# facebook/facebook360_dep

Hardware: AMD Instinct MI355X
Metric: depth Mpix/s per GPU (full pyramid, 16-cam 2048^2 rig); % HBM-read roofline (higher is better)
Workload: dtype f32+f64; 1 GPU; BASELINE config 3: 16-camera 2048x2048 synthetic rig, 8-frame sequence, full 10-level pyramid per frame, per-level temporal filter (+-2 frames); the same sequence for every --gpus N (block partition, 8 frame(s) on this rank); rig=cfg2, cameras=16, frames=8, temporal_filter=True, halo_transport=local, parallelism=frames x1

## Files before the change

facebook360_dep_amd/csrc/derp_camera.h:

```cpp
#pragma once
#include <hip/hip_runtime.h>
#include <math.h>
#include <stdint.h>

#include "../../include/derp_hip.h"

#define DERP_HD __host__ __device__ __forceinline__

namespace derp {

struct Cam {
  double pos[3];
  double R[9];
  double principal[2];
  double focal[2];
  double dist[3];
  double dist_max;
  double cos_fov;
  double edge_sq;
  int32_t type;
  int32_t default_fov;
  int32_t dist_zero;
  int32_t pad;
};

struct D2 {
  double x, y;
};
struct D3 {
  double x, y, z;
};

DERP_HD double sum3(double a, double b, double c) {
  return a + (b + c);
}

DERP_HD double distort_factor(const Cam& c, double r2) {
  double result = c.dist[2];
  result = c.dist[1] + r2 * result;
  result = c.dist[0] + r2 * result;
  return 1.0 + r2 * result;
}
DERP_HD double distort(const Cam& c, double r) {
  r = (c.dist_max < r) ? c.dist_max : r;
  return distort_factor(c, r * r) * r;
}

DERP_HD double undistort(const Cam& c, const double y) {
  if (c.dist_zero) {
    return y;
  }
  if (y >= distort(c, c.dist_max)) {
    return c.dist_max;
  }
  const double smidgen = 1.0 / 1e4;
  double x0 = 0, y0 = 0, dy0 = 1;
  for (int step = 0; step < 10; ++step) {
    const double x1 = (y - y0) / dy0 + x0;
    const double y1 = distort(c, x1);
    if (fabs(y1 - y) < smidgen) {
      return x1;
    }
    const double dy1 = (distort(c, x1 + smidgen) - y1) / smidgen;
    x0 = x1;
    y0 = y1;
    dy0 = dy1;
  }
  return x0;
}

static constexpr int kAtanLutDoubles = 20;
#if defined(__HIP_DEVICE_COMPILE__)
__device__ __forceinline__ double div_plain(double n, double d) {
  double r = __builtin_amdgcn_rcp(d);
  r = __builtin_fma(__builtin_fma(-d, r, 1.0), r, r);
  r = __builtin_fma(__builtin_fma(-d, r, 1.0), r, r);
  const double q = n * r;
// ... 145 lines not shown
    if (p.z < 0) {
      const double n = DERP_SQRT(sum3(p.x * p.x, p.y * p.y, p.z * p.z));
      px = p.x / n;
      py = p.y / n;
    } else {
      const double n = DERP_SQRT(p.x * p.x + p.y * p.y);
      px = p.x / n;
      py = p.y / n;
    }
    const double f = distort_factor(c, px * px + py * py);
    return {f * px, f * py};
  }
}

#undef DERP_SQRT
DERP_HD D3 sensor_to_camera(const Cam& c, const D2& s) {
  const double sq = s.x * s.x + s.y * s.y;
  if (sq == 0) {
    return {0, 0, -1};
  }
  const double norm = sqrt(sq);
  const double r = undistort(c, norm);
  double theta;
  if (c.type == DERP_FTHETA) {
    theta = r;
  } else if (c.type == DERP_RECTILINEAR) {
    theta = atan(r);
  } else if (c.type == DERP_EQUISOLID) {
    theta = r <= 2 ? 2 * asin(r / 2) : M_PI;
  } else {
    theta = r <= 1 ? asin(r) : M_PI / 2;
  }
  const double k = sin(theta) / norm;
  return {k * s.x, k * s.y, -cos(theta)};
}

DERP_HD D3 rig_direction(const Cam& c, double px, double py, double prx, double pry, double fx, double fy) {
  const D2 sensor = {(px - prx) / fx, (py - pry) / fy};
  const D3 u = sensor_to_camera(c, sensor);
  return {
      sum3(c.R[0] * u.x, c.R[3] * u.y, c.R[6] * u.z),
      sum3(c.R[1] * u.x, c.R[4] * u.y, c.R[7] * u.z),
      sum3(c.R[2] * u.x, c.R[5] * u.y, c.R[8] * u.z)};
}

DERP_HD bool outside_image_circle(const Cam& c, double px, double py, double prx, double pry, double fx, double fy) {
  if (c.default_fov) {
    return false;
  }
  const double sx = (px - prx) / fx, sy = (py - pry) / fy;
  return sx * sx + sy * sy >= c.edge_sq;
}

template <int LEAN = 0>
DERP_HD bool sees(const Cam& c, const D3& rig, double prx, double pry, double fx, double fy,
                  double resx, double resy, D2& pix, const double* atanLut = nullptr) {
  const D3 v = {rig.x - c.pos[0], rig.y - c.pos[1], rig.z - c.pos[2]};
  const double back = sum3(c.R[6] * v.x, c.R[7] * v.y, c.R[8] * v.z);
  if (c.cos_fov != -1) {
    if (c.cos_fov == 0) {
      if (back >= 0) {
        return false;
      }
    } else {
      const double dot = -back;
      const double sq = sum3(v.x * v.x, v.y * v.y, v.z * v.z);
      if (dot * fabs(dot) <= c.cos_fov * fabs(c.cos_fov) * sq) {
        return false;
      }
    }
  }
  const D3 cam = {
      sum3(c.R[0] * v.x, c.R[1] * v.y, c.R[2] * v.z),
      sum3(c.R[3] * v.x, c.R[4] * v.y, c.R[5] * v.z),
      back};
  const D2 s = camera_to_sensor<LEAN>(c, cam, atanLut);
  pix.x = fx * s.x + prx;
  pix.y = fy * s.y + pry;
  return !(0 > pix.x || pix.x >= resx || 0 > pix.y || pix.y >= resy);
}

inline double host_poly(const double* k, int deg, double x) {
  double acc = k[deg];
  for (int i = deg; i-- > 0;) {
    acc = acc * x + k[i];
  }
  return acc;
}

inline double host_smallest_positive_root(const double* k, int deg) {
  double stops[4];
  int n_stops = 0;
  if (deg == 3) {
    const double a = 3 * k[3], b = 2 * k[2], c = k[1];
    const double disc = b * b - 4 * a * c;
    if (disc >= 0) {
      const double q = -0.5 * (b + copysign(sqrt(disc), b));
      double r0 = q / a, r1 = (q != 0) ? c / q : r0;
      if (r0 > r1) {
        const double t = r0;
        r0 = r1;
        r1 = t;
      }
      if (r0 > 0) {
        stops[n_stops++] = r0;
      }
      if (r1 > 0 && r1 != r0) {
        stops[n_stops++] = r1;
      }
    }
  } else if (deg == 2) {
    const double r = -k[1] / (2 * k[2]);
    if (r > 0) {
      stops[n_stops++] = r;
    }
  }
  double left = 0, f_left = k[0];
  for (int seg = 0; seg <= n_stops; ++seg) {
    double right;
    if (seg < n_stops) {
      right = stops[seg];
    } else {
// ... 121 lines not shown
    c.R[3] = t + sz;
    t = c1x * az;
    c.R[2] = t + sy;
    c.R[6] = t - sy;
    t = c1y * az;
    c.R[5] = t - sx;
    c.R[7] = t + sx;
    c.R[0] = c1x * ax + cs;
    c.R[4] = c1y * ay + cs;
    c.R[8] = c1z * az + cs;
  }
  double res[2] = {j.resolution[0], j.resolution[1]};
  double pr[2] = {j.has_principal ? j.principal[0] : res[0] / 2, j.has_principal ? j.principal[1] : res[1] / 2};
  c.dist[0] = c.dist[1] = c.dist[2] = 0;
  c.dist_max = INFINITY;
  if (j.has_distortion) {
    int count = 3;
    while (count > 0 && j.distortion[count - 1] == 0) {
      --count;
    }
    if (count > 0) {
      double k[4] = {1, 0, 0, 0};
      for (int i = 0; i < count; ++i) {
        k[i + 1] = j.distortion[i] * (2 * i + 3);
      }
      const double y = host_smallest_positive_root(k, count);
      for (int i = 0; i < 3; ++i) {
        c.dist[i] = j.distortion[i];
      }
      c.dist_max = sqrt(y);
    }
  }
  c.dist_zero = (c.dist[0] == 0 && c.dist[1] == 0 && c.dist[2] == 0);
  const double def_cos = (j.type == DERP_RECTILINEAR || j.type == DERP_ORTHOGRAPHIC) ? 0.0 : -1.0;
  if (j.has_fov) {
    c.cos_fov = cos(j.fov);
    if (!(c.cos_fov >= def_cos)) {
      return "fov exceeds the camera type's default";
    }
  } else {
    c.cos_fov = def_cos;
  }
  c.default_fov = (c.cos_fov == def_cos);
  c.principal[0] = pr[0] / res[0];
  c.principal[1] = pr[1] / res[1];
  c.focal[0] = j.focal[0] / res[0];
  c.focal[1] = j.focal[1] / res[1];
  c.edge_sq = 0;
  if (!c.default_fov) {
    const double sin_fov = sqrt(1 - c.cos_fov * c.cos_fov);
    const D2 e = camera_to_sensor(c, D3{0, sin_fov, -c.cos_fov});
    c.edge_sq = e.x * e.x + e.y * e.y;
  }
  c.pad = 0;
  return nullptr;
}

}
```

facebook360_dep_amd/csrc/derp_capi.hip:

```cpp
#include <hip/hip_runtime.h>

#include <algorithm>
#include <cfloat>
#include <cmath>
#include <cstdarg>
#include <cstdio>
#include <cstdlib>
#include <cstring>
#include <map>
#include <memory>
#include <string>
#include <vector>

#include <rocprim/device/device_radix_sort.hpp>

#include "../../include/derp_hip.h"
#include "derp_host.h"
#include "derp_kernels.h"
#include "derp_mesh.h"
#include "derp_points.h"
#include "derp_render.h"
#include "derp_geometric.h"
#include "derp_sweep.h"
#include "derp_align.h"
// ... 1073 lines not shown
  (void)hipMemcpy(c->camsSrc.p, c->camsSrcH.data(), sizeof(Cam) * n_src, hipMemcpyHostToDevice);
  (void)hipMemcpy(c->camsDst.p, c->camsDstH.data(), sizeof(Cam) * n_dst, hipMemcpyHostToDevice);
  (void)hipMemcpy(c->dst2src.p, c->dst2srcH.data(), sizeof(int) * n_dst, hipMemcpyHostToDevice);
  (void)hipMemset(c->counters.p, 0, c->counters.bytes);
  *out = owner.release();
  return 0;
}

void derp_destroy(derp_ctx* c) {
  if (!c) {
    return;
  }
  (void)hipSetDevice(c->device);
  (void)hipStreamSynchronize(c->stream);
  for (auto& l : c->lanes) {
    (void)hipStreamSynchronize(l->stream);
  }
  drain_spans(c);
  for (auto& l : c->lanes) {
    (void)hipStreamDestroy(l->stream);
    (void)hipEventDestroy(l->done);
  }
  if (c->laneReady) {
    (void)hipEventDestroy(c->laneReady);
  }
  (void)hipStreamDestroy(c->stream);
  (void)hipStreamDestroy(c->copyStream);
  delete c;
}

const char* derp_last_error(const derp_ctx* c) {
  return c ? c->err.c_str() : g_create_error.c_str();
}

int derp_set_options(derp_ctx* c, const derp_options* o) {
  if (!c || !o) {
    return 1;
  }
  if (o->random_proposals < 0) {
    return fail(c, "Check failed: random_proposals >= 0");
  }
  c->opt = *o;
  return 0;
}

int derp_set_pyramid(derp_ctx* c, int num_levels, const int* widths, const int* heights, int width_full,
                     int height_full) {
  if (!c) {
    return 1;
  }
  if (num_levels <= 0 || num_levels > kMaxLevels) {
    return fail(c, "num_levels %d out of range (1..%d)", num_levels, kMaxLevels);
  }
  HIPCHK(c, hipSetDevice(c->device));
  c->numLevels = num_levels;
  c->widthFull = width_full;
  c->heightFull = height_full;
  c->LW.assign(widths, widths + num_levels);
  c->LH.assign(heights, heights + num_levels);
  c->frames.clear();
  c->frames.resize(1);
  c->curSlot = 0;
  TRY(alloc_pyramid(c, c->frame()));
  size_t nmax = 0;
  for (int l = 0; l < num_levels; ++l) {
    nmax = std::max(nmax, npx(c, l));
  }
  TRY(alloc_work_set(c, c->w, nmax));
  ALLOC(c, c->fovMask, nmax * c->D);
  c->cur = -1;
  c->warpCachedLevel = -1;
  c->fovCachedLevel = -1;
  HIPCHK(c, hipStreamSynchronize(c->stream));
  return 0;
}

int derp_set_frame_slots(derp_ctx* c, int n_slots) {
  if (!c || c->numLevels == 0) {
    return fail(c, "derp_set_pyramid has not been called");
  }
  if (n_slots < 1 || n_slots > 4096) {
    return fail(c, "n_slots %d out of range (1..4096)", n_slots);
  }
  HIPCHK(c, hipSetDevice(c->device));
  TRY(select_frame(c, 0));
  const int had = (int)c->frames.size();
  c->frames.resize(n_slots);
  for (int k = had; k < n_slots; ++k) {
    TRY(alloc_pyramid(c, c->frames[k]));
  }
  HIPCHK(c, hipStreamSynchronize(c->stream));
  return 0;
}

int derp_select_frame(derp_ctx* c, int slot) {
  if (!c || c->numLevels == 0) {
    return fail(c, "derp_set_pyramid has not been called");
  }
  return select_frame(c, slot);
}

int derp_frame_slots(const derp_ctx* c, int* n_slots, int* selected) {
  if (!c) {
    return 1;
  }
  if (n_slots) {
// ... 327 lines not shown
```

facebook360_dep_amd/csrc/derp_debug_api.h:

```cpp
#pragma once

namespace {
struct HostPairs {
  SsdPair* p;
  SsdPair get(int i) const {
    return p[i];
  }
  void set(int i, const SsdPair& v) {
    p[i] = v;
  }
};
int stage_index(const char* stage) {
  for (int i = 0; i < ST_COUNT; ++i) {
    if (strcmp(stage, kStageNames[i]) == 0) {
      return i;
    }
  }
  return -1;
}
}

int derp_debug_atan2_ypos(derp_ctx* c, const double* y, const double* x, double* out, size_t n) {
  if (!c || !y || !x || !out) {
    return fail(c, "bad arguments");
  }
  ALLOC(c, c->w.staging, 3 * n * sizeof(double));
  double* d = c->w.staging.as<double>();
  HIPCHK(c, hipMemcpyAsync(d, y, n * sizeof(double), hipMemcpyHostToDevice, c->stream));
  HIPCHK(c, hipMemcpyAsync(d + n, x, n * sizeof(double), hipMemcpyHostToDevice, c->stream));
  hipLaunchKernelGGL(k_debug_atan2_ypos, dim3(flat_grid(n)), dim3(256), 0, c->stream, d, d + n, d + 2 * n, n);
  KCHECK(c);
  HIPCHK(c, hipMemcpyAsync(out, d + 2 * n, n * sizeof(double), hipMemcpyDeviceToHost, c->stream));
  HIPCHK(c, hipStreamSynchronize(c->stream));
  return 0;
}

int derp_debug_fp64(derp_ctx* c, int op, const double* a, const double* b, double* out, size_t n) {
  if (!c || !a || !out || op < 0 || op > 3 || (op >= 2 && !b)) {
    return fail(c, "bad arguments");
  }
  if (n == 0) {
    return 0;
  }
  ALLOC(c, c->w.staging, 3 * n * sizeof(double));
  double* d = c->w.staging.as<double>();
  HIPCHK(c, hipMemcpyAsync(d, a, n * sizeof(double), hipMemcpyHostToDevice, c->stream));
  HIPCHK(c, hipMemcpyAsync(d + n, op >= 2 ? b : a, n * sizeof(double), hipMemcpyHostToDevice, c->stream));
  hipLaunchKernelGGL(k_debug_fp64, dim3(flat_grid(n)), dim3(256), 0, c->stream, op, d, d + n, d + 2 * n, n);
  KCHECK(c);
  HIPCHK(c, hipMemcpyAsync(out, d + 2 * n, n * sizeof(double), hipMemcpyDeviceToHost, c->stream));
  HIPCHK(c, hipStreamSynchronize(c->stream));
  return 0;
}

int derp_debug_expf(derp_ctx* c, int mode, const float* x, float* out, size_t n) {
  if (!c || !x || !out || mode < 0 || mode > 1) {
    return fail(c, "bad arguments");
  }
  if (n == 0) {
    return 0;
  }
  ALLOC(c, c->w.staging, 2 * n * sizeof(float));
  float* d = c->w.staging.as<float>();
  HIPCHK(c, hipMemcpyAsync(d, x, n * sizeof(float), hipMemcpyHostToDevice, c->stream));
  hipLaunchKernelGGL(k_debug_expf, dim3(flat_grid(n)), dim3(256), 0, c->stream, mode, d, d + n, n);
  KCHECK(c);
  HIPCHK(c, hipMemcpyAsync(out, d + n, n * sizeof(float), hipMemcpyDeviceToHost, c->stream));
  HIPCHK(c, hipStreamSynchronize(c->stream));
  return 0;
}

int derp_debug_sees(derp_ctx* c, int src, const double* xyz, size_t n, double* out) {
  if (!c || !xyz || !out || src < 0 || src >= c->S) {
    return fail(c, "bad arguments");
  }
  if (n == 0) {
    return 0;
  }
  ALLOC(c, c->w.staging, 9 * n * sizeof(double));
  double* d = c->w.staging.as<double>();
  HIPCHK(c, hipMemcpyAsync(d, xyz, 3 * n * sizeof(double), hipMemcpyHostToDevice, c->stream));
  hipLaunchKernelGGL(k_debug_sees, dim3(flat_grid(n)), dim3(256), 0, c->stream, c->camsSrc.as<Cam>(), src, d, d + 3 * n, n);
  KCHECK(c);
  HIPCHK(c, hipMemcpyAsync(out, d + 3 * n, 6 * n * sizeof(double), hipMemcpyDeviceToHost, c->stream));
  HIPCHK(c, hipStreamSynchronize(c->stream));
  return 0;
}

int derp_debug_download(derp_ctx* c, int d, int s, int which, void* out) {
  TRY(need_current(c, false));
  const int L = c->cur;
  const int W = c->LW[L], H = c->LH[L];
  const size_t n = (size_t)W * H;
  HIPCHK(c, hipStreamSynchronize(c->stream));
  if (which == 4) {
    HIPCHK(c, hipMemcpy(out, c->w.srcVar.as<float>() + (size_t)s * n, n * sizeof(float), hipMemcpyDeviceToHost));
    return 0;
  }
  if (which == 5) {
    HIPCHK(c, hipMemcpy(out, c->fovMask.as<uint8_t>() + (size_t)d * n, n, hipMemcpyDeviceToHost));
    return 0;
  }
  if (which == 9) {
    if (s < 0 || s >= c->S) {
      return fail(c, "bad source index");
    }
    std::vector<ushort4> tmp(n);
    HIPCHK(c, hipMemcpy(tmp.data(), c->w.ownBias.as<ushort4>() + (size_t)s * n, n * sizeof(ushort4), hipMemcpyDeviceToHost));
    uint16_t* o = reinterpret_cast<uint16_t*>(out);
// ... 286 lines not shown
```

facebook360_dep_amd/csrc/derp_kernels.h:

```cpp
#pragma once
#include <hip/hip_runtime.h>
#include <math.h>
#include <stdint.h>

#include <type_traits>

#include "derp_camera.h"
#include "gcc_algos.h"

namespace derp {

#ifndef DERP_COST_MIN_WAVES
#define DERP_COST_MIN_WAVES 4
#endif
#ifndef DERP_RANDOM_MIN_WAVES
#define DERP_RANDOM_MIN_WAVES 4
#endif
#ifndef DERP_RANDOM_TILED
#define DERP_RANDOM_TILED 0
#endif
#ifndef DERP_MIX_HOT_ONLY
#define DERP_MIX_HOT_ONLY 0
#endif
#ifndef DERP_PHASE_TIMERS
// ... 159 lines not shown

struct LdsPairs {
  SsdPair* base;
  int stride;
  const double* atanLut;
  __device__ __forceinline__ SsdPair get(int i) const {
    return base[i * stride];
  }
  __device__ __forceinline__ void set(int i, const SsdPair& v) {
    base[i * stride] = v;
  }
};

__device__ __forceinline__ LdsPairs cost_wave_prologue(const LevelView& V, int d, int x0, int y0, PatchWin*& win) {
  extern __shared__ SsdPair ldsPairs[];
  __shared__ PatchWin patchWin[kCostBlock / 64];
  win = &patchWin[threadIdx.x >> 6];
  patch_window_fill(V, V.dst2src[d], x0, y0, win);
#if defined(__HIP_DEVICE_COMPILE__)
  __shared__ double atanLut[kAtanLutDoubles];
  atan_lut_fill(atanLut);
  LdsPairs pairs{ldsPairs + threadIdx.x, (int)blockDim.x, atanLut};
#else
  LdsPairs pairs{ldsPairs + threadIdx.x, (int)blockDim.x, nullptr};
#endif
  __syncthreads();
  return pairs;
}
__device__ __forceinline__ LdsPairs cost_block_prologue(PatchWin*& win) {
  static_assert(kCostBlock == 64, "a wave leaves an empty tile on its own: the block must be that one wave");
  extern __shared__ SsdPair ldsPairs[];
  __shared__ PatchWin patchWin[kCostBlock / 64];
  win = &patchWin[threadIdx.x >> 6];
#if defined(__HIP_DEVICE_COMPILE__)
  __shared__ double atanLut[kAtanLutDoubles];
  return LdsPairs{ldsPairs + threadIdx.x, (int)blockDim.x, atanLut};
#else
  return LdsPairs{ldsPairs + threadIdx.x, (int)blockDim.x, nullptr};
#endif
}
__device__ __forceinline__ void cost_tile_prologue(const LevelView& V, int d, int x0, int y0, PatchWin* win, const LdsPairs& pairs,
                                                   bool& lutReady) {
  __syncthreads();
  patch_window_fill(V, V.dst2src[d], x0, y0, win);
#if defined(__HIP_DEVICE_COMPILE__)
  if (!lutReady) {
    atan_lut_fill(const_cast<double*>(pairs.atanLut));
    lutReady = true;
  }
#endif
  __syncthreads();
}

struct SsdTexels {
  u4a8 raw[4][2];
  u4a8 ba, bb;
};
template <bool TILED>
__device__ __forceinline__ void ssd_issue_random(const LevelView& V, const ushort4* __restrict__ col, const ushort4* __restrict__ colT,
                                                 const ushort4* __restrict__ bia, float xDstSrc, float yDstSrc, SsdTexels& T,
                                                 bool& border) {
  const int pitch = V.W + 2 * kPadC;
  const int xi = (int)roundf(xDstSrc), yi = (int)roundf(yDstSrc);
  const unsigned off = ((unsigned)(yi - 2 + kPadC) * (unsigned)pitch + (unsigned)(xi - 2 + kPadC)) * 8u;
  if constexpr (TILED) {
    const unsigned xa = (unsigned)(xi - 2 + kPadC), ya = (unsigned)(yi - 2 + kPadC);
    const unsigned rowTiles = (unsigned)tiled_tiles_x(V.W) * 128u;
    const unsigned xr = xa & 3u, yr = ya & 3u;
    const unsigned base0 = (ya >> 2) * rowTiles + (xa >> 2) * 128u + yr * 32u + xr * 8u;
    const char* base = reinterpret_cast<const char*>(colT);
    typedef unsigned int u2 __attribute__((ext_vector_type(2)));
#pragma unroll
    for (int row = 0; row < 4; ++row) {
      const unsigned ro = base0 + (unsigned)row * 32u + ((yr + (unsigned)row > 3u) ? rowTiles - 128u : 0u);
#pragma unroll
      for (int k = 0; k < 4; ++k) {
        const unsigned o = ro + (unsigned)k * 8u + ((xr + (unsigned)k > 3u) ? 96u : 0u);
        const u2 t = *reinterpret_cast<const u2*>(base + o);
        if (k & 1) {
          T.raw[row][k >> 1].z = t.x;
          T.raw[row][k >> 1].w = t.y;
        } else {
          T.raw[row][k >> 1].x = t.x;
          T.raw[row][k >> 1].y = t.y;
        }
      }
    }
  } else {
    const char* base = reinterpret_cast<const char*>(col);
#pragma unroll
    for (int row = 0; row < 4; ++row) {
      T.raw[row][0] = *reinterpret_cast<const u4a8*>(base + (off + (unsigned)row * (unsigned)pitch * 8u));
      T.raw[row][1] = *reinterpret_cast<const u4a8*>(base + (off + (unsigned)row * (unsigned)pitch * 8u + 16u));
    }
  }
  border = xi < 2 || yi < 2 || xi > V.W - 2 || yi > V.H - 2;
  T.ba = T.bb = (u4a8){0u, 0u, 0u, 0u};
  if (border) {
    const unsigned boff = off + ((unsigned)pitch + 1u) * 8u;
    const char* bbase = reinterpret_cast<const char*>(bia);
    T.ba = *reinterpret_cast<const u4a8*>(bbase + boff);
    T.bb = *reinterpret_cast<const u4a8*>(bbase + (boff + (unsigned)pitch * 8u));
  }
}
__device__ __forceinline__ void ssd_issue(const LevelView& V, const ushort4* __restrict__ col,
                                          const ushort4* __restrict__ bia, float xDstSrc, float yDstSrc, SsdTexels& T) {
  const int pitch = V.W + 2 * kPadC;
  const int xi = (int)roundf(xDstSrc), yi = (int)roundf(yDstSrc);
  const unsigned off = ((unsigned)(yi - 2 + kPadC) * (unsigned)pitch + (unsigned)(xi - 2 + kPadC)) * 8u;
  const char* base = reinterpret_cast<const char*>(col);
#pragma unroll
  for (int row = 0; row < 4; ++row) {
    T.raw[row][0] = *reinterpret_cast<const u4a8*>(base + (off + (unsigned)row * (unsigned)pitch * 8u));
    T.raw[row][1] = *reinterpret_cast<const u4a8*>(base + (off + (unsigned)row * (unsigned)pitch * 8u + 16u));
  }
  const unsigned boff = off + ((unsigned)pitch + 1u) * 8u;
  const char* bbase = reinterpret_cast<const char*>(bia);
  T.ba = *reinterpret_cast<const u4a8*>(bbase + boff);
  T.bb = *reinterpret_cast<const u4a8*>(bbase + (boff + (unsigned)pitch * 8u));
}

template <bool RANDOM>
__device__ __forceinline__ SsdPair ssd_arith(const LevelView& V, const PixCtx& px, const ushort4* __restrict__ col,
                                             const SsdTexels& T, float xDstSrc, float yDstSrc, bool border = true) {
  const int pitch = V.W + 2 * kPadC;
  const u4a8 (&raw)[4][2] = T.raw;
  auto word_bg = [&](const u4a8 (&q)[4][2], int r, int k) { return (k & 1) ? q[r][k >> 1].z : q[r][k >> 1].x; };
  auto word_r = [&](const u4a8 (&q)[4][2], int r, int k) { return (k & 1) ? q[r][k >> 1].w : q[r][k >> 1].y; };
  float bias[3];
  const float bxf = roundf(xDstSrc), byf = roundf(yDstSrc);
  const float bxw = xDstSrc - bxf + 0.5f, byw = yDstSrc - byf + 0.5f;
  const float w00 = (1 - bxw) * (1 - byw), w01 = bxw * (1 - byw), w10 = (1 - bxw) * byw, w11 = bxw * byw;
  if constexpr (RANDOM) {
    float top[3][2], bot[3][2];
#pragma unroll
    for (int k = 3; k >= 0; --k) {
      float c[3][4];
#pragma unroll
      for (int r = 0; r < 4; ++r) {
        const unsigned bg = word_bg(raw, r, k), rr = word_r(raw, r, k);
        c[0][r] = (float)(bg & 0xffff);
        c[1][r] = (float)(bg >> 16);
        c[2][r] = (float)(rr & 0xffff);
      }
#pragma unroll
      for (int ch = 0; ch < 3; ++ch) {
        const float m = c[ch][1] + c[ch][2];
        const float vT = m + c[ch][0], vB = m + c[ch][3];
        if (k == 3) {
          top[ch][1] = vT + 4.0f;
          bot[ch][1] = vB + 4.0f;
        } else if (k == 2) {
          top[ch][1] += vT;
          bot[ch][1] += vB;
          top[ch][0] = vT + 4.0f;
          bot[ch][0] = vB + 4.0f;
        } else if (k == 1) {
          top[ch][1] += vT;
          bot[ch][1] += vB;
          top[ch][0] += vT;
          bot[ch][0] += vB;
        } else {
          top[ch][0] += vT;
          bot[ch][0] += vB;
        }
      }
    }
    const float ninth = 1.0f / 9.0f;
#pragma unroll
    for (int ch = 0; ch < 3; ++ch) {
      const float t00 = __builtin_truncf(top[ch][0] * ninth), t01 = __builtin_truncf(top[ch][1] * ninth);
      const float t10 = __builtin_truncf(bot[ch][0] * ninth), t11 = __builtin_truncf(bot[ch][1] * ninth);
      bias[ch] = px.dstBias(ch) - bilerp_u16(t00, t01, t10, t11, w00, w01, w10, w11);
    }
    if (__ballot(border) != 0ull) {
      if (border) {
        const u4a8 a = T.ba, b = T.bb;
        bias[0] = px.dstBias(0) - bilerp_u16((float)(a.x & 0xffff), (float)(a.z & 0xffff), (float)(b.x & 0xffff), (float)(b.z & 0xffff), w00, w01, w10, w11);
        bias[1] = px.dstBias(1) - bilerp_u16((float)(a.x >> 16), (float)(a.z >> 16), (float)(b.x >> 16), (float)(b.z >> 16), w00, w01, w10, w11);
        bias[2] = px.dstBias(2) - bilerp_u16((float)(a.y & 0xffff), (float)(a.w & 0xffff), (float)(b.y & 0xffff), (float)(b.w & 0xffff), w00, w01, w10, w11);
      }
    }
  } else {
// ... 72 lines not shown
    const v2f biasBG = (v2f){bias[0], bias[1]};
    const v2f omyp = splat2(1.0f) - ywp;
    const float omym = 1 - ywm;
    ColF lo, hi;
    unpack(0, lo);
#pragma unroll
    for (int ix = 0; ix < 3; ++ix) {
      unpack(ix + 1, hi);
      const float omx = 1 - xw[ix];
      const v2f w00p = splat2(omx) * omyp, w01p = splat2(xw[ix]) * omyp, w10p = splat2(omx) * ywp, w11p = splat2(xw[ix]) * ywp;
      const float w00m = omx * omym, w01m = xw[ix] * omym, w10m = omx * ywm, w11m = xw[ix] * ywm;
      float bgd0[3], bgd1[3];
#pragma unroll
      for (int iy = 0; iy < 3; ++iy) {
        const float w00 = iy == 1 ? w00m : iy == 0 ? w00p.x : w00p.y;
        const float w01 = iy == 1 ? w01m : iy == 0 ? w01p.x : w01p.y;
        const float w10 = iy == 1 ? w10m : iy == 0 ? w10p.x : w10p.y;
        const float w11 = iy == 1 ? w11m : iy == 0 ? w11p.x : w11p.y;
        const v2f v = splat2(w00) * lo.bg[iy] + splat2(w01) * hi.bg[iy] + splat2(w10) * lo.bg[iy + 1] +
                      splat2(w11) * hi.bg[iy + 1];
        const v2f db = px.patchBG(ix, iy) - trunc2(v);
        const v2f dn = db - biasBG;
        const v2f s0 = db * db, s1 = dn * dn;
        float t0 = s0.x + s0.y, t1 = s1.x + s1.y;
        asm("" : "+v"(t0), "+v"(t1));
        bgd0[iy] = t0;
        bgd1[iy] = t1;
      }
      v2f e0, e1;
      {
        const v2f v = w00p * lo.rE + w01p * hi.rE + w10p * lo.rO + w11p * hi.rO;
        const v2f db = (v2f){px.patchR(ix, 0), px.patchR(ix, 2)} - trunc2(v);
        const v2f dn = db - splat2(bias[2]);
        e0 = (v2f){bgd0[0], bgd0[2]} + db * db;
        e1 = (v2f){bgd1[0], bgd1[2]} + dn * dn;
      }
      float m0, m1;
      {
        const float v = w00m * lo.rO.x + w01m * hi.rO.x + w10m * lo.rE.y + w11m * hi.rE.y;
        const float db = px.patchR(ix, 1) - __builtin_truncf(v);
        const float dn = db - bias[2];
        m0 = bgd0[1] + db * db;
        m1 = bgd1[1] + dn * dn;
      }
      first += e0.x;
      first += m0;
      first += e0.y;
      second += e1.x;
      second += m1;
      second += e1.y;
      lo = hi;
    }
  };
  const float xfc = roundf(xDstSrc), yfc = roundf(yDstSrc);
  const bool exact = (xDstSrc >= 1.0f) && (yDstSrc >= 1.0f) && ((xDstSrc + 1.0f) - 1.0f == xDstSrc) &&
                     ((yDstSrc + 1.0f) - 1.0f == yDstSrc);
  int xi[3], yi[3];
  float xw[3], yw[3];
  bool regular = true;
  xi[1] = (int)xfc;
  yi[1] = (int)yfc;
  xw[0] = xw[1] = xw[2] = xDstSrc - xfc + 0.5f;
  yw[0] = yw[1] = yw[2] = yDstSrc - yfc + 0.5f;
  if (!exact) {
#pragma unroll
    for (int k = 0; k < 3; k += 2) {
      const float xs = xDstSrc + (float)(k - 1), ys = yDstSrc + (float)(k - 1);
      const float xf = roundf(xs), yf = roundf(ys);
      xi[k] = (int)xf;
      yi[k] = (int)yf;
      xw[k] = xs - xf + 0.5f;
      yw[k] = ys - yf + 0.5f;
    }
    regular = (xi[0] == xi[1] - 1) && (xi[2] == xi[1] + 1) && (yi[0] == yi[1] - 1) && (yi[2] == yi[1] + 1);
  }
  if (!RANDOM && __ballot(!exact) == 0ull) {
    const float xwu[3] = {xw[1], xw[1], xw[1]};
    block_packed(xwu, splat2(yw[1]), yw[1]);
  } else if (regular) {
    if constexpr (RANDOM) {
      block_scalar(xw, yw);
    } else {
      block_packed(xw, (v2f){yw[0], yw[2]}, yw[1]);
    }
  } else if (DERP_MIX_HOT_ONLY) {
    first = second = 0.f;
  } else {
    for (int ix = 0; ix < 3; ++ix) {
      for (int iy = 0; iy < 3; ++iy) {
        const float w00 = (1 - xw[ix]) * (1 - yw[iy]), w01 = xw[ix] * (1 - yw[iy]);
        const float w10 = (1 - xw[ix]) * yw[iy], w11 = xw[ix] * yw[iy];
        const int x0 = min(max(xi[ix] - 1, -kPadC), V.W + kPadC - 1), x1 = min(max(xi[ix], -kPadC), V.W + kPadC - 1);
        const int y0 = min(max(yi[iy] - 1, -kPadC), V.H + kPadC - 1), y1 = min(max(yi[iy], -kPadC), V.H + kPadC - 1);
        const ushort4 q00 = col[(size_t)(y0 + kPadC) * pitch + x0 + kPadC];
        const ushort4 q01 = col[(size_t)(y0 + kPadC) * pitch + x1 + kPadC];
        const ushort4 q10 = col[(size_t)(y1 + kPadC) * pitch + x0 + kPadC];
        const ushort4 q11 = col[(size_t)(y1 + kPadC) * pitch + x1 + kPadC];
        const float p00[3] = {(float)q00.x, (float)q00.y, (float)q00.z};
        const float p01[3] = {(float)q01.x, (float)q01.y, (float)q01.z};
        const float p10[3] = {(float)q10.x, (float)q10.y, (float)q10.z};
        const float p11[3] = {(float)q11.x, (float)q11.y, (float)q11.z};
        const v2f pbg = px.winBG[iy * kWinW + ix];
        const float pch[3] = {pbg.x, pbg.y, px.winR[iy * kWinW + ix]};
        float d0 = 0.f, d1 = 0.f;
        for (int c = 0; c < 3; ++c) {
          const float cs = bilerp_u16(p00[c], p01[c], p10[c], p11[c], w00, w01, w10, w11);
          const float db = pch[c] - cs;
// ... 95 lines not shown
  if constexpr (RELOAD_RAY) {
    unsigned i = pix;
    asm("" : "+v"(i) : "v"(disparity));
    const double* rd = V.rayDir + (size_t)(V.dst0 + dl) * ((size_t)V.W * V.H);
    if constexpr (RANDOM) {
      rayD = {at32(rd, i), at32(rd + V.rayStride, i), at32(rd + 2 * V.rayStride, i)};
    } else {
      rayD = {rd[i], rd[V.rayStride + i], rd[2 * V.rayStride + i]};
    }
  }
  const D3 pWorld = {px.rayO.x + rayD.x * depth, px.rayO.y + rayD.y * depth, px.rayO.z + rayD.z * depth};
  const size_t wPlane = warp_plane(V), cPlane = color_plane(V);
  const int wPitch = V.W + 2 * kPadW;
  unsigned mask = 0, waveMask = 0;
  cull = __builtin_amdgcn_readfirstlane(__ballot(!(depth >= kCullMinDepth)) != 0ull ? 0u : cull);
  const ushort4* colBase = V.projColor + (size_t)dl * (V.S - 1) * cPlane;
  const ushort4* biaBase = V.projBias + (size_t)dl * (V.S - 1) * cPlane;
  const size_t tPlane = tiled_plane(V.W, V.H);
  const ushort4* colTBase = RANDOM ? V.projColorT + (size_t)dl * (V.S - 1) * tPlane : nullptr;
  {
    bool pend = false;
    int pendSlot = 0;
    f4a8 pa = {0, 0, 0, 0}, pb = {0, 0, 0, 0};
    float pxw = 0, pyw = 0;
    auto consume = [&]() {
      const float w00 = (1 - pxw) * (1 - pyw), w01 = pxw * (1 - pyw), w10 = (1 - pxw) * pyw, w11 = pxw * pyw;
      const float wx = bilerp_f(pa.x, pa.z, pb.x, pb.z, w00, w01, w10, w11);
      const float wy = bilerp_f(pa.y, pa.w, pb.y, pb.w, w00, w01, w10, w11);
      const float xDstSrc = wx + 0.5f, yDstSrc = wy + 0.5f;
      const bool ok = pend && !(isnan(xDstSrc) || isnan(yDstSrc));
      if (ok) {
        pairs.set(pendSlot, SsdPair{xDstSrc, yDstSrc});
        mask |= 1u << pendSlot;
      }
      if (__ballot(ok) != 0ull) {
        waveMask |= 1u << pendSlot;
      }
    };
    for (int s = 0; s < V.S; ++s) {
      if (s == own || ((cull >> slot(s, own)) & 1u)) {
        continue;
      }
      const Cam& cs = V.camsSrc[s];
      D2 pn;
      const bool vis = sees<cost_sees_lean<RANDOM>()>(cs, pWorld, cs.principal[0], cs.principal[1], cs.focal[0], cs.focal[1],
                                                      1.0, 1.0, pn, pairs.atanLut);
      if (__ballot(pend) != 0ull) {
        consume();
      }
      pend = vis;
      pendSlot = slot(s, own);
      if (__ballot(vis) != 0ull) {
        const float sx = (float)(pn.x * V.Wd), sy = (float)(pn.y * V.Hd);
        const float xf = roundf(sx), yf = roundf(sy);
        const int xi = (int)xf, yi = (int)yf;
        pxw = sx - xf + 0.5f;
        pyw = sy - yf + 0.5f;
        const size_t tab = (size_t)dl * (V.S - 1) + pendSlot;
        const char* wbase = reinterpret_cast<const char*>(V.projWarp + tab * wPlane);
        const unsigned woff = vis ? ((unsigned)(yi - 1 + kPadW) * (unsigned)wPitch + (unsigned)(xi - 1 + kPadW)) * 8u : 0u;
        pa = *reinterpret_cast<const f4a8*>(wbase + woff);
        pb = *reinterpret_cast<const f4a8*>(wbase + (woff + (unsigned)wPitch * 8u));
      }
    }
    if (__ballot(pend) != 0ull) {
      consume();
    }
  }
  const unsigned tc1 = phase_clock();
  const int ssdCount = __popc(mask);
  nPair += ssdCount;
#ifdef DERP_COUNT_UNION
  if (slots) {
    *slots += __popc(__builtin_amdgcn_readfirstlane(waveMask));
  }
#endif
  int keep = 1;
  if (ssdCount < keep) {
    return make_float2(3.402823466e+38f, 0.0f);
  }
  {
    int cnt = 0;
    for (unsigned wm = __builtin_amdgcn_readfirstlane(waveMask); wm != 0; wm &= wm - 1) {
      const int t = __builtin_ctz(wm);
      if ((mask >> t) & 1) {
        const SsdPair e = pairs.get(t);
        const SsdPair ssd = compute_ssd<RANDOM>(V, px, colBase + (size_t)t * cPlane, biaBase + (size_t)t * cPlane, e.first,
                                                        e.second, RANDOM ? colTBase + (size_t)t * tPlane : nullptr);
        pairs.set(cnt, ssd);
        ++cnt;
      }
    }
  }
  const unsigned tc2 = phase_clock();
  keep = max(keep, ssdCount - 2);
  GccSelect<LdsPairs> sel(pairs);
  sel.nth_element(keep, ssdCount);
  float cost = 0;
  for (int i = 0; i < keep; ++i) {
    cost += pairs.get(i).second;
  }
  cost /= (float)keep;
  const float trustCoef = 1.0f / (float)keep;
  float confidence = px.confidence;
  if constexpr (RELOAD_RAY) {
    unsigned i = pix;
    asm("" : "+v"(i) : "v"(cost));
// ... 1365 lines not shown
__device__ __forceinline__ float expf_glibc_poly(float x, const unsigned long long* tab) {
  const double InvLn2N = 0x1.71547652b82fep+0 * 32;
  const double C0 = 0x1.c6af84b912394p-5 / 32 / 32 / 32, C1 = 0x1.ebfce50fac4f3p-3 / 32 / 32,
               C2 = 0x1.62e42ff0c52d6p-1 / 32;
  const double SHIFT = 0x1.8p+52;
  const double xd = (double)x;
  double kd = __builtin_fma(InvLn2N, xd, SHIFT);
  const unsigned long long ki = (unsigned long long)__double_as_longlong(kd);
  kd -= SHIFT;
  const double r = __builtin_fma(InvLn2N, xd, -kd);
  const unsigned long long t = tab[ki & 31] + (ki << 47);
  const double sc = __longlong_as_double((long long)t);
  const double z = __builtin_fma(C0, r, C1);
  const double r2 = r * r;
  double y = __builtin_fma(C2, r, 1.0);
  y = __builtin_fma(z, r2, y);
  y = y * sc;
  return (float)y;
}

__device__ __forceinline__ float expf_glibc(float x, const unsigned long long* tab) {
  const unsigned abstop = (__float_as_uint(x) >> 20) & 0x7ff;
  if (abstop >= (0x42b00000u >> 20)) {
    if (__float_as_uint(x) == 0xff800000u) {
      return 0.0f;
    }
    if (abstop >= (0x7f800000u >> 20)) {
      return x + x;
    }
    if (x > 0x1.62e42ep6f) {
      return __builtin_inff();
    }
    if (x < -0x1.9fe368p6f) {
      return 0.0f;
    }
  }
  return expf_glibc_poly(x, tab);
}

__device__ __forceinline__ float expf_glibc_nonpos(float x, const unsigned long long* tab) {
  if (x < -0x1.9fe368p6f) {
    return 0.0f;
  }
  return expf_glibc_poly(x, tab);
}

__global__ void __launch_bounds__(256) k_debug_expf(int mode, const float* __restrict__ x, float* __restrict__ out, size_t n) {
  __shared__ unsigned long long expTab[32];
  if (threadIdx.x < 32) {
    expTab[threadIdx.x] = kExp2fTab[threadIdx.x];
  }
  __syncthreads();
  for (size_t i = (size_t)blockIdx.x * blockDim.x + threadIdx.x; i < n; i += (size_t)gridDim.x * blockDim.x) {
    out[i] = mode == 0 ? expf_glibc(x[i], expTab) : expf_glibc_nonpos(x[i], expTab);
  }
}

template <bool GUIDE_U16>
__device__ __forceinline__ float4 bilateral_texel(const void* __restrict__ guideV, size_t j, float value) {
  if (GUIDE_U16) {
    const ushort4 g = reinterpret_cast<const ushort4*>(guideV)[j];
    const float factor = 1 / 65535.0f;
    return make_float4(g.x * factor, g.y * factor, g.z * factor, value);
  }
  const float* g = reinterpret_cast<const float*>(guideV) + j * 3;
  const float factor = 1 / 1.0f;
  return make_float4(g[0] * factor, g[1] * factor, g[2] * factor, value);
}

__device__ __forceinline__ void bilateral_tap(float4 centre, float4 t, float weight0, float weight1, float weight2,
                                              double rcpDenom, const unsigned long long* expTab, float& sumWeight,
                                              float& weightedAvg) {
  const float d0 = centre.x - t.x, d1 = centre.y - t.y, d2 = centre.z - t.z;
  const float colorDiffSq = weight0 * (d0 * d0) + weight1 * (d1 * d1) + weight2 * (d2 * d2);
  const float weight = expf_glibc(div_by_const(div_by_const(-colorDiffSq, 1.0 / 3.0), rcpDenom), expTab);
  sumWeight += weight;
  weightedAvg += weight * t.w;
}

__device__ __forceinline__ void bilateral_tap_fast(float4 centre, float4 t, float weight0, double rcpDenom,
                                                   const unsigned long long* expTab, float& sumWeight, float& weightedAvg) {
  const float d0 = centre.x - t.x, d1 = centre.y - t.y, d2 = centre.z - t.z;
  const float colorDiffSq = weight0 * (d0 * d0) + (d1 * d1) + (d2 * d2);
  const float weight = expf_glibc_nonpos(div_by_const(div_by_const(-colorDiffSq, 1.0 / 3.0), rcpDenom), expTab);
  sumWeight += weight;
  weightedAvg += weight * t.w;
}

template <bool GUIDE_U16, bool FAST_TAP = false>
__global__ void __launch_bounds__(256)
    k_joint_bilateral(const float* __restrict__ image, const void* __restrict__ guideV,
                      const uint8_t* __restrict__ mask, int W, int H, int radius, float sigma, float weight0,
                      float weight1, float weight2, float* __restrict__ out, size_t planeStride, size_t guideStride,
                      const int* __restrict__ guideIndex) {
  static_assert(GUIDE_U16 || !FAST_TAP, "the fast tap's range argument needs the u16 guide");
  extern __shared__ float ldsTile[];
  __shared__ unsigned long long expTab[32];
  if (threadIdx.x < 32) {
    expTab[threadIdx.x] = kExp2fTab[threadIdx.x];
  }
  const int p = blockIdx.z;
  const int T = 16 + 2 * radius;
  const int P = (T + 15) & ~15;
  const int n = P * T;
  float4* tTex = reinterpret_cast<float4*>(ldsTile);
  uint8_t* tMask = reinterpret_cast<uint8_t*>(ldsTile + 4 * n);
  const float* img = image + (size_t)p * planeStride;
// ... 1292 lines not shown
```

facebook360_dep_amd/derp.py:

```python
import ctypes as C
import os

import numpy as np

_HERE = os.path.dirname(os.path.abspath(__file__))
LIB_PATH = os.environ.get("DERP_LIB") or os.path.join(_HERE, "libderp_hip.so")
CAM_TYPES = {"FTHETA": 0, "RECTILINEAR": 1, "EQUISOLID": 2, "ORTHOGRAPHIC": 3}

STAGES = ["fov_mask", "variance", "own_bias", "upsample", "proj_warp", "reproject", "proj_bias", "brute_force",
          "random_proposals", "ping_pong", "mismatches", "bilateral", "median", "mask_fov", "temporal"]


class SeqOptions(C.Structure):
    _fields_ = [
        ("time_radius", C.c_int32), ("sigma", C.c_float), ("weight_b", C.c_float), ("weight_g", C.c_float),
        ("weight_r", C.c_float), ("space_radius", C.c_int32), ("use_foreground_masks", C.c_int32),
        ("partition", C.c_int32), ("do_temporal_filter", C.c_int32), ("resident_frames", C.c_int32),
    ]


class SeqTransfer(C.Structure):
    _fields_ = [("frame", C.c_int32), ("from_rank", C.c_int32), ("to_rank", C.c_int32)]


# ... 336 lines not shown

    def level_begin(self, level):
        self._cur = level
        self._ck(lib().derp_level_begin(self.h, level))

    def stage(self, name):
        fn = {
            "reproject_colors": "derp_stage_reproject_colors", "brute_force": "derp_stage_brute_force",
            "random_proposals": "derp_stage_random_proposals", "ping_pong": "derp_stage_ping_pong",
            "mismatches": "derp_stage_mismatches", "bilateral": "derp_stage_bilateral_filter", "median": "derp_stage_median_filter",
            "mask_fov": "derp_stage_mask_fov", "end": "derp_level_end",
        }[name]
        self._ck(getattr(lib(), fn)(self.h))

    def set_level_disparity(self, d, disp):
        disp = np.ascontiguousarray(disp, dtype=np.float32)
        self._ck(lib().derp_set_level_disparity(self.h, d, _p(disp)))

    def get_level_disparity(self, d):
        out = np.zeros(self._shape(self._cur), dtype=np.float32)
        self._ck(lib().derp_get_level_disparity(self.h, d, _p(out)))
        return out

    def cost_map(self, d, disp):
        disp = np.ascontiguousarray(disp, dtype=np.float32)
        cost = np.zeros(self._shape(self._cur), dtype=np.float32)
        conf = np.zeros(self._shape(self._cur), dtype=np.float32)
        self._ck(lib().derp_cost_map(self.h, d, _p(disp), _p(cost), _p(conf)))
        return cost, conf

    def debug_atan2_ypos(self, y, x):
        y = np.ascontiguousarray(y, np.float64)
        x = np.ascontiguousarray(x, np.float64)
        out = np.zeros_like(y)
        self._ck(lib().derp_debug_atan2_ypos(self.h, _p(y), _p(x), _p(out), C.c_size_t(y.size)))
        return out

    FP64_OPS = {"sqrt_lean": 0, "sqrt": 1, "div_plain": 2, "div": 3}

    def debug_fp64(self, op, a, b=None):
        a = np.ascontiguousarray(a, np.float64)
        b = None if b is None else np.ascontiguousarray(b, np.float64)
        assert b is None or b.shape == a.shape
        out = np.zeros_like(a)
        self._ck(lib().derp_debug_fp64(self.h, self.FP64_OPS[op], _p(a), _p(b), _p(out), C.c_size_t(a.size)))
        return out

    def debug_expf(self, x, nonpos=False):
        x = np.ascontiguousarray(x, np.float32)
        out = np.zeros_like(x)
        self._ck(lib().derp_debug_expf(self.h, int(bool(nonpos)), _p(x), _p(out), C.c_size_t(x.size)))
        return out

    def debug_sees(self, src, xyz):
        xyz = np.ascontiguousarray(xyz, np.float64).reshape(-1, 3)
        out = np.zeros((len(xyz), 2, 3))
        self._ck(lib().derp_debug_sees(self.h, src, _p(xyz), C.c_size_t(len(xyz)), _p(out)))
        return out[:, :, 0].T != 0, np.ascontiguousarray(out[:, :, 1:].transpose(1, 0, 2))

    def debug(self, d, s, which):
        h, w = self._shape(self._cur)
        spec = {"warp": (0, (h, w, 2), np.float32), "color": (2, (h, w, 3), np.uint16),
                "bias": (3, (h, w, 3), np.uint16), "variance": (4, (h, w), np.float32),
                "fov": (5, (h, w), np.uint8),
                "color_padded": (6, (h + 4, w + 4, 4), np.uint16), "bias_padded": (7, (h + 4, w + 4, 4), np.uint16),
                "tile_seen": (8, ((h + 31) // 32, (w + 31) // 32), np.uint8),
                "own_bias": (9, (h, w, 3), np.uint16), "rank": (10, (h, w), np.uint32)}[which]
        out = np.zeros(spec[1], dtype=spec[2])
        self._ck(lib().derp_debug_download(self.h, d, s, spec[0], _p(out)))
        return out

    def mismatch_mask(self, d):
        out = np.zeros(self._shape(self._cur), dtype=np.uint8)
        self._ck(lib().derp_download_mismatch_mask(self.h, d, _p(out)))
        return out

    def layer_disparities(self, fg, bg):
        fg = np.ascontiguousarray(fg, dtype=np.float32)
        bg = np.ascontiguousarray(bg, dtype=np.float32)
        out = np.zeros(fg.shape, dtype=np.uint8)
        self._ck(lib().derp_layer_disparities(self.h, _p(fg), _p(bg), C.c_size_t(fg.size), _p(out)))
        return out

    def ssim(self, x, y, blur_radius=1, alpha=1.0, beta=1.0, gamma=1.0):
        x = np.ascontiguousarray(x, dtype=np.float32)
        y = np.ascontiguousarray(y, dtype=np.float32)
        h, w = x.shape[:2]
        out = np.zeros((h, w, 3), dtype=np.float32)
        self._ck(lib().derp_ssim(self.h, _p(x), _p(y), w, h, blur_radius, C.c_float(alpha), C.c_float(beta),
                                 C.c_float(gamma), _p(out)))
        return out

    def rephotograph(self, target, colors, disps):
        colors = [np.ascontiguousarray(c, dtype=np.uint16) for c in colors]
        disps = [np.ascontiguousarray(d, dtype=np.float32) for d in disps]
        h, w = disps[0].shape
        cp = (C.c_void_p * len(colors))(*[c.ctypes.data for c in colors])
        dp = (C.c_void_p * len(disps))(*[d.ctypes.data for d in disps])
        out = np.zeros((h, w, 4), dtype=np.float32)
        self._ck(lib().derp_rephotograph(self.h, target, cp, dp, w, h, _p(out)))
        return out

    def rephotograph_upload(self, colors, disps):
        colors = [np.ascontiguousarray(c, dtype=np.uint16) for c in colors]
        disps = [np.ascontiguousarray(d, dtype=np.float32) for d in disps]
        h, w = disps[0].shape
# ... 778 lines not shown
```

Before: 534.1 Mpix/s.

## Add cheap cone-visibility prefilter and faster positive round-half-away in SSD sampling

Precomputes a per-camera cone classification and a slightly inflated cosine factor so the device-side sees() test can, for narrow FOV cones, accept most points with a cheap L1-norm bound. The exact squared-norm check runs only for lanes the bound cannot decide, using a wave ballot. Separately, roundf is replaced with trunc(x + just-under-half), which matches round-half-away only for non-negative inputs, so a size limit on pyramid levels is added. A debug hook exposes the new rounding for testing. The cost is more branching and reliance on coordinates being non-negative.

```diff
diff --git a/facebook360_dep_amd/csrc/derp_camera.h b/facebook360_dep_amd/csrc/derp_camera.h
--- a/facebook360_dep_amd/csrc/derp_camera.h
+++ b/facebook360_dep_amd/csrc/derp_camera.h
@@ -18,11 +18,13 @@
   double dist_max;
   double cos_fov;
   double edge_sq;
+  double cone_kappa;
   int32_t type;
   int32_t default_fov;
   int32_t dist_zero;
-  int32_t pad;
+  int32_t cone_kind;
 };
+enum { kConeNone = 0, kConeHalfSpace = 1, kConeNarrow = 2, kConeWide = 3 };
 
 struct D2 {
   double x, y;
@@ -274,22 +276,51 @@
   return sx * sx + sy * sy >= c.edge_sq;
 }
 
+DERP_HD bool outside_cone(const Cam& c, const D3& v, double dot) {
+  const double sq = sum3(v.x * v.x, v.y * v.y, v.z * v.z);
+  return dot * fabs(dot) <= c.cos_fov * fabs(c.cos_fov) * sq;
+}
+
 template <int LEAN = 0>
 DERP_HD bool sees(const Cam& c, const D3& rig, double prx, double pry, double fx, double fy,
                   double resx, double resy, D2& pix, const double* atanLut = nullptr) {
   const D3 v = {rig.x - c.pos[0], rig.y - c.pos[1], rig.z - c.pos[2]};
   const double back = sum3(c.R[6] * v.x, c.R[7] * v.y, c.R[8] * v.z);
+#if defined(__HIP_DEVICE_COMPILE__)
+  if (LEAN & 3) {
+    if (c.cone_kind == kConeHalfSpace) {
+      if (back >= 0) {
+        return false;
+      }
+    } else if (c.cone_kind == kConeWide) {
+      if (outside_cone(c, v, -back)) {
+        return false;
+      }
+    } else if (c.cone_kind == kConeNarrow) {
+      const double dot = -back;
+      if (dot <= 0) {
+        return false;
+      }
+      const double t = c.cone_kappa * (fabs(v.x) + (fabs(v.y) + fabs(v.z)));
+      const unsigned long long sure = __builtin_amdgcn_fcmp(dot, t, 2);
+      const unsigned long long unsure = __builtin_amdgcn_ballot_w64(true) & ~sure;
+      if (unsure != 0ull) {
+        if (__builtin_amdgcn_inverse_ballot_w64(unsure)) {
+          if (outside_cone(c, v, dot)) {
+            return false;
+          }
+        }
+      }
+    }
+  } else
+#endif
   if (c.cos_fov != -1) {
     if (c.cos_fov == 0) {
       if (back >= 0) {
         return false;
       }
-    } else {
-      const double dot = -back;
-      const double sq = sum3(v.x * v.x, v.y * v.y, v.z * v.z);
-      if (dot * fabs(dot) <= c.cos_fov * fabs(c.cos_fov) * sq) {
-        return false;
-      }
+    } else if (outside_cone(c, v, -back)) {
+      return false;
     }
   }
   const D3 cam = {
@@ -517,7 +548,8 @@
     const D2 e = camera_to_sensor(c, D3{0, sin_fov, -c.cos_fov});
     c.edge_sq = e.x * e.x + e.y * e.y;
   }
-  c.pad = 0;
+  c.cone_kappa = c.cos_fov * (1.0 + 0x1.0p-20);
+  c.cone_kind = c.cos_fov == -1 ? kConeNone : c.cos_fov == 0 ? kConeHalfSpace : c.cos_fov >= 0x1.0p-100 ? kConeNarrow : kConeWide;
   return nullptr;
 }
 
diff --git a/facebook360_dep_amd/csrc/derp_capi.hip b/facebook360_dep_amd/csrc/derp_capi.hip
--- a/facebook360_dep_amd/csrc/derp_capi.hip
+++ b/facebook360_dep_amd/csrc/derp_capi.hip
@@ -1149,6 +1149,11 @@
   if (num_levels <= 0 || num_levels > kMaxLevels) {
     return fail(c, "num_levels %d out of range (1..%d)", num_levels, kMaxLevels);
   }
+  for (int l = 0; l < num_levels; ++l) {
+    if (widths[l] >= (1 << 22) || heights[l] >= (1 << 22)) {
+      return fail(c, "level %d is too large (%dx%d, a side may be 4194303 at most)", l, widths[l], heights[l]);
+    }
+  }
   HIPCHK(c, hipSetDevice(c->device));
   c->numLevels = num_levels;
   c->widthFull = width_full;
diff --git a/facebook360_dep_amd/csrc/derp_debug_api.h b/facebook360_dep_amd/csrc/derp_debug_api.h
--- a/facebook360_dep_amd/csrc/derp_debug_api.h
+++ b/facebook360_dep_amd/csrc/derp_debug_api.h
@@ -54,7 +54,7 @@
 }
 
 int derp_debug_expf(derp_ctx* c, int mode, const float* x, float* out, size_t n) {
-  if (!c || !x || !out || mode < 0 || mode > 1) {
+  if (!c || !x || !out || mode < 0 || mode > 2) {
     return fail(c, "bad arguments");
   }
   if (n == 0) {
diff --git a/facebook360_dep_amd/csrc/derp_kernels.h b/facebook360_dep_amd/csrc/derp_kernels.h
--- a/facebook360_dep_amd/csrc/derp_kernels.h
+++ b/facebook360_dep_amd/csrc/derp_kernels.h
@@ -235,6 +235,10 @@
   __syncthreads();
 }
 
+__device__ __forceinline__ float round_half_away_pos(float x) {
+  return __builtin_truncf(x + 0x1.fffffep-2f);
+}
+
 struct SsdTexels {
   u4a8 raw[4][2];
   u4a8 ba, bb;
@@ -244,7 +248,7 @@
                                                  const ushort4* __restrict__ bia, float xDstSrc, float yDstSrc, SsdTexels& T,
                                                  bool& border) {
   const int pitch = V.W + 2 * kPadC;
-  const int xi = (int)roundf(xDstSrc), yi = (int)roundf(yDstSrc);
+  const int xi = (int)round_half_away_pos(xDstSrc), yi = (int)round_half_away_pos(yDstSrc);
   const unsigned off = ((unsigned)(yi - 2 + kPadC) * (unsigned)pitch + (unsigned)(xi - 2 + kPadC)) * 8u;
   if constexpr (TILED) {
     const unsigned xa = (unsigned)(xi - 2 + kPadC), ya = (unsigned)(yi - 2 + kPadC);
@@ -289,7 +293,7 @@
 __device__ __forceinline__ void ssd_issue(const LevelView& V, const ushort4* __restrict__ col,
                                           const ushort4* __restrict__ bia, float xDstSrc, float yDstSrc, SsdTexels& T) {
   const int pitch = V.W + 2 * kPadC;
-  const int xi = (int)roundf(xDstSrc), yi = (int)roundf(yDstSrc);
+  const int xi = (int)round_half_away_pos(xDstSrc), yi = (int)round_half_away_pos(yDstSrc);
   const unsigned off = ((unsigned)(yi - 2 + kPadC) * (unsigned)pitch + (unsigned)(xi - 2 + kPadC)) * 8u;
   const char* base = reinterpret_cast<const char*>(col);
 #pragma unroll
@@ -311,7 +315,7 @@
   auto word_bg = [&](const u4a8 (&q)[4][2], int r, int k) { return (k & 1) ? q[r][k >> 1].z : q[r][k >> 1].x; };
   auto word_r = [&](const u4a8 (&q)[4][2], int r, int k) { return (k & 1) ? q[r][k >> 1].w : q[r][k >> 1].y; };
   float bias[3];
-  const float bxf = roundf(xDstSrc), byf = roundf(yDstSrc);
+  const float bxf = round_half_away_pos(xDstSrc), byf = round_half_away_pos(yDstSrc);
   const float bxw = xDstSrc - bxf + 0.5f, byw = yDstSrc - byf + 0.5f;
   const float w00 = (1 - bxw) * (1 - byw), w01 = bxw * (1 - byw), w10 = (1 - bxw) * byw, w11 = bxw * byw;
   if constexpr (RANDOM) {
@@ -490,7 +494,7 @@
       lo = hi;
     }
   };
-  const float xfc = roundf(xDstSrc), yfc = roundf(yDstSrc);
+  const float xfc = round_half_away_pos(xDstSrc), yfc = round_half_away_pos(yDstSrc);
   const bool exact = (xDstSrc >= 1.0f) && (yDstSrc >= 1.0f) && ((xDstSrc + 1.0f) - 1.0f == xDstSrc) &&
                      ((yDstSrc + 1.0f) - 1.0f == yDstSrc);
   int xi[3], yi[3];
@@ -692,7 +696,7 @@
       pendSlot = slot(s, own);
       if (__ballot(vis) != 0ull) {
         const float sx = (float)(pn.x * V.Wd), sy = (float)(pn.y * V.Hd);
-        const float xf = roundf(sx), yf = roundf(sy);
+        const float xf = round_half_away_pos(sx), yf = round_half_away_pos(sy);
         const int xi = (int)xf, yi = (int)yf;
         pxw = sx - xf + 0.5f;
         pyw = sy - yf + 0.5f;
@@ -2164,7 +2168,7 @@
   }
   __syncthreads();
   for (size_t i = (size_t)blockIdx.x * blockDim.x + threadIdx.x; i < n; i += (size_t)gridDim.x * blockDim.x) {
-    out[i] = mode == 0 ? expf_glibc(x[i], expTab) : expf_glibc_nonpos(x[i], expTab);
+    out[i] = mode == 2 ? round_half_away_pos(x[i]) : mode == 0 ? expf_glibc(x[i], expTab) : expf_glibc_nonpos(x[i], expTab);
   }
 }
 
diff --git a/facebook360_dep_amd/derp.py b/facebook360_dep_amd/derp.py
--- a/facebook360_dep_amd/derp.py
+++ b/facebook360_dep_amd/derp.py
@@ -412,6 +412,12 @@
         self._ck(lib().derp_debug_expf(self.h, int(bool(nonpos)), _p(x), _p(out), C.c_size_t(x.size)))
         return out
 
+    def debug_round_half_away(self, x):
+        x = np.ascontiguousarray(x, np.float32)
+        out = np.zeros_like(x)
+        self._ck(lib().derp_debug_expf(self.h, 2, _p(x), _p(out), C.c_size_t(x.size)))
+        return out
+
     def debug_sees(self, src, xyz):
         xyz = np.ascontiguousarray(xyz, np.float64).reshape(-1, 3)
         out = np.zeros((len(xyz), 2, 3))
```

Measured after the change: 541.3 Mpix/s (median of 6 runs). +1.3%, better.
